# AnnaLew/pangenomix

Hardware: AMD Instinct MI355X
Metric: proteins/sec clustered at 0.8 identity + pan/core iters/sec, 400-genome set (higher is better)
Workload: dtype i32

## Files before the change

pangenomix_amd/csrc/cluster.hip:

```cpp
#include <algorithm>
#include <chrono>
#include <cstdlib>
#include <cmath>
#include <type_traits>
#include <functional>
#include <condition_variable>
#include <mutex>
#include <thread>
#include <vector>

#include "cluster_layout.h"
#include "cluster_resolve.h"
#include "cluster_tables.h"
#include "pgx_internal.h"

namespace {

using namespace pgxc;

constexpr uint32_t kWindowMax = 65536;
constexpr int kDiscoveryRounds = 2;
constexpr uint32_t kBlockCap = 4096;
constexpr uint32_t kBlockCapMin = 64;

// ... 39 lines not shown
    const uint8_t *res;
    const uint64_t *off;
    const uint32_t *len;
    const uint32_t *wcode;
    const uint16_t *wmult;
    const uint32_t *wcnt;
    const uint32_t *pk;
    const uint32_t *pk_off;
    uint32_t n_fwd;
    int32_t base;
    int32_t kd;
    int32_t nt;
    uint32_t mshift;
};
__device__ __forceinline__ uint32_t entry_rmask(const DevSeqs &S) { return (1u << S.mshift) - 1u; }
__device__ __forceinline__ uint32_t entry_fmax(const DevSeqs &S) { return 0xFFFFFFFFu >> S.mshift; }
__device__ __forceinline__ uint32_t real_of(const DevSeqs &S, uint32_t k) { return k >= S.n_fwd ? k - S.n_fwd : k; }

__constant__ int8_t kAa2Idx_dev[26] = {0, 2, 4, 3, 6, 13, 7, 8, 9, 20, 11, 10, 12,
                                       2, 20, 14, 5, 1, 15, 16, 20, 19, 17, 20, 18, 6};

__device__ __forceinline__ bool is_letter(uint8_t ch) {
    ch &= 0xDF;
    return ch >= 'A' && ch <= 'Z';
}

__global__ __launch_bounds__(256) void seq_len_kernel(const uint8_t *__restrict__ res,
                                                     const uint64_t *__restrict__ off, uint32_t n, uint64_t total,
                                                     uint32_t *__restrict__ len) {
    const uint32_t lane = threadIdx.x & 63u;
    const uint32_t i = blockIdx.x * 4u + (threadIdx.x >> 6);
    if (i >= n) return;
    const uint64_t b = off[i], e = off[i + 1];
    uint32_t c = 0;
    const uint64_t a0 = b & ~3ull;
    for (uint64_t a = a0 + 4ull * lane; a < e; a += 256) {
        uint32_t word = 0;
        if (a + 4 <= total) word = *reinterpret_cast<const uint32_t *>(res + a);
        else for (uint64_t p = a; p < total; ++p) word |= (uint32_t)res[p] << (8 * (p - a));
#pragma unroll
        for (int t = 0; t < 4; ++t) {
            const uint64_t p = a + t;
            c += (p >= b && p < e) && is_letter((uint8_t)(word >> (8 * t)));
        }
    }
    for (int d = 32; d > 0; d >>= 1) c += __shfl_xor(c, d);
    if (lane == 0) len[i] = c;
}

__global__ __launch_bounds__(256) void encode_gather_kernel(const uint8_t *__restrict__ in,
                                                           const uint64_t *__restrict__ in_off,
                                                           const uint32_t *__restrict__ order,
                                                           const uint64_t *__restrict__ out_off,
                                                           uint8_t *__restrict__ out, uint32_t n, int nt) {
    const uint32_t lane = threadIdx.x & 63u;
    const uint32_t k = blockIdx.x * 4u + (threadIdx.x >> 6);
    if (k >= n) return;
    const uint32_t src = order[k];
    const uint64_t b = in_off[src], e = in_off[src + 1];
    uint64_t w = out_off[k];
    for (uint64_t q0 = b; q0 < e; q0 += 256) {
        uint8_t chs[4];
#pragma unroll
        for (int j = 0; j < 4; ++j) { const uint64_t p = q0 + 64u * j + lane; chs[j] = p < e ? in[p] : (uint8_t)0; }
#pragma unroll
        for (int j = 0; j < 4; ++j) {
            const uint8_t ch = chs[j];
            const bool ok = is_letter(ch);
            const unsigned long long m = __ballot(ok);
            if (ok) {
                const uint8_t up = ch & 0xDF;
                const uint8_t idx = nt ? (uint8_t)(up == 'A' ? 0 : up == 'C' ? 1 : up == 'G' ? 2 : (up == 'T' || up == 'U') ? 3 : 4)
                                       : (uint8_t)kAa2Idx_dev[up - 'A'];
                out[w + __popcll(m & ((1ull << lane) - 1ull))] = idx;
            }
            w += __popcll(m);
        }
    }
}

__global__ __launch_bounds__(256) void revcomp_kernel(uint8_t *__restrict__ res, const uint64_t *__restrict__ off,
                                                     const uint32_t *__restrict__ len, uint32_t n) {
    const uint32_t lane = threadIdx.x & 63u;
    const uint32_t k = blockIdx.x * 4u + (threadIdx.x >> 6);
    if (k >= n) return;
    const uint64_t src = off[k], dst = off[n + k];
    const uint32_t L = len[k];
    for (uint32_t i = lane; i < L; i += 64) {
        const uint8_t b = res[src + L - 1 - i];
        res[dst + i] = b < 4 ? (uint8_t)(3 - b) : b;
    }
}

__global__ __launch_bounds__(256) void pack5_kernel(const uint8_t *__restrict__ res, const uint64_t *__restrict__ off,
                                                   const uint32_t *__restrict__ len,
                                                   const uint32_t *__restrict__ pk_off, uint32_t n,
                                                   uint32_t *__restrict__ pk) {
    const uint32_t lane = threadIdx.x & 63u;
    const uint32_t k = blockIdx.x * 4u + (threadIdx.x >> 6);
    if (k >= n) return;
    const uint8_t *s = res + off[k];
    const uint32_t L = len[k], nw = (L + 5u) / 6u;
    uint32_t *dst = pk + pk_off[k];
    for (uint32_t w = lane; w < nw; w += 64) {
        uint32_t x = 0;
        for (uint32_t t = 0; t < 6; ++t)
            if (6 * w + t < L) x |= (uint32_t)s[6 * w + t] << (5u * t);
        dst[w] = x;
    }
}

constexpr uint32_t kDevSortMaxLen = 65535;
constexpr uint32_t kHistLds = 4096;
constexpr uint32_t kSortShare = 1024;
constexpr uint32_t kSortCells = 4u << 20;
constexpr uint32_t kScanTile = 2048;
enum : uint32_t { H_OVER = 0, H_MAX = 1, H_BINS = 4 };

constexpr int kClearSegs = 6;
struct ClearArgs { uint32_t *p[kClearSegs]; uint32_t words[kClearSegs]; int n; uint32_t *one; };
__global__ __launch_bounds__(256) void clear_kernel(ClearArgs a) {
    const uint32_t t = blockIdx.x * 256u + threadIdx.x, step = gridDim.x * 256u;
    for (int s = 0; s < a.n; ++s)
        for (uint32_t i = t; i < a.words[s]; i += step) a.p[s][i] = 0u;
    if (a.one && t == 0) *a.one = 1u;
}

__global__ __launch_bounds__(1024) void len_hist_kernel(const uint32_t *__restrict__ len, uint32_t n, int32_t min_length,
                                                       uint32_t *__restrict__ hist) {
    __shared__ uint32_t h[kHistLds];
    for (uint32_t b = threadIdx.x; b < kHistLds; b += 1024u) h[b] = 0u;
    __syncthreads();
    uint32_t mx = 0, over = 0;
    for (uint32_t i = blockIdx.x * 1024u + threadIdx.x; i < n; i += gridDim.x * 1024u) {
        const uint32_t L = len[i];
        mx = max(mx, L);
        if (L > kDevSortMaxLen) { ++over; continue; }
        if ((int32_t)L <= min_length) continue;
        if (L < kHistLds) atomicAdd(&h[L], 1u);
        else atomicAdd(&hist[H_BINS + L], 1u);
    }
    for (int d = 32; d > 0; d >>= 1) { mx = max(mx, (uint32_t)__shfl_xor(mx, d)); over += __shfl_xor(over, d); }
    if ((threadIdx.x & 63u) == 0) {
        if (mx) atomicMax(&hist[H_MAX], mx);
        if (over) atomicAdd(&hist[H_OVER], over);
    }
    __syncthreads();
    for (uint32_t b = threadIdx.x; b < kHistLds; b += 1024u)
        if (h[b]) atomicAdd(&hist[H_BINS + b], h[b]);
}

__global__ __launch_bounds__(256) void sort_count_kernel(const uint32_t *__restrict__ len, uint32_t n, int32_t min_length,
                                                        uint32_t max_len, uint32_t per, uint32_t n_shares,
// ... 1888 lines not shown
    hipEvent_t strike = nullptr, post = nullptr;
    WindowSet(pgx_ctx *c, DevSlot counters, DevSlot best, DevSlot flags, DevSlot pairs, DevSlot gscratch, PinSlot w,
              PinSlot b, PinSlot cnt)
        : counters_buf(c, counters), best_buf(c, best), flags_buf(c, flags), pairs_buf(c, pairs), gscratch_buf(c, gscratch),
          hW(c, w), h_best(c, b), h_ccnt(c, cnt) {}
    WindowSet(const WindowSet &) = delete;
    WindowSet &operator=(const WindowSet &) = delete;
    ~WindowSet() {
        if (strike) (void)hipEventDestroy(strike);
        if (post) (void)hipEventDestroy(post);
    }
};

struct PendingWindow {
    bool pending = false;
    uint32_t b0 = 0, nb = 0, nW = 0;
    bool sweep = false;
    int set = 0;
    uint64_t window_words = 0;
    Pinned<Pair> *hW = nullptr;
    Pinned<unsigned long long> *h_best = nullptr;
    Pinned<uint32_t> *h_ccnt = nullptr;
};

struct ClusterCall {
    pgx_ctx *ctx;
    const pgx_cluster_params *P;
    hipStream_t st_main;
    const uint8_t *d_residues = nullptr;
    const uint64_t *d_offsets = nullptr;
    uint32_t n_in = 0;
    uint64_t total_in = 0;
    int32_t *out_cluster = nullptr, *out_member = nullptr;
    float *out_identity = nullptr;
    uint8_t *out_strand = nullptr;
    bool want_stats = false;
    bool nt, both, overlap, exchanging, native_exchange, count_replicated;
    uint32_t shard_index, shard_count;
    bool trace, trace2;
    unsigned nth = 1;
    Clock::time_point t_call0, t_loop0;
    double t_mark = 0.0, t_resolve = 0.0, t_close = 0.0;
    bool dev_sort = false, need_gscratch = false, chunking = false;
    uint32_t n = 0, nv = 0, max_len = 0, n_runs = 0, mshift = 8, n_codes = 1, bm_words = 0;
    uint32_t window_cap = 0, pair_cap_k = 0, packed_len = 0, diag_grid = 0, gs_stride = 0, gs_cells = 0, tag_stride = 1;
    uint64_t total = 0, total_pk = 0, max_window_words = 0;
    double thr_frac = 0.0;
    const uint32_t *len_hist = nullptr;
    std::vector<uint32_t> host_hist;
    uint64_t *run_off = nullptr;
    uint32_t *run_pos = nullptr, *run_pk = nullptr;
    std::vector<uint32_t> flush_at;
    DevSeqs DS{};
    uint32_t pair_cap = 4u << 20;
    uint32_t block_cap = 0;
    int pool_cur = 0;
    uint64_t pool_cap = 0;
    uint32_t epoch_idx = 0;
    uint32_t epoch_tag = 0;
    double cur_frac = 0.0;
    uint64_t chunk_words = 0;
    uint64_t pending_words = 0;
    PendingWindow pending;
    DevBuf d_res, d_off, d_len, d_wcode, d_wmult, d_wcnt, d_aa1, d_aas, d_aan, d_lines, d_pool[2], d_idx, d_newbits, d_touched,
        d_first, d_rcvis, d_visits, d_pairsK, d_blk_list, d_ulist, d_new_list, d_order, d_list, d_gather, d_pk, d_pkoff, d_thr,
        d_hugewords, d_xsend, d_xrecv,
        d_hist, d_sortcnt, d_tilesum, d_runs, d_in_len;
    WindowSet sets[2];
    unsigned long long *x_send = nullptr;
    const unsigned long long *x_recv = nullptr;
    HostVec<uint32_t> h_hist, order, h_len, h_wcnt;
    HostVec<uint64_t> h_off, h_runs;
    HostVec<int32_t> h_thr;
    HostVec<int32_t> cluster_of;
    HostVec<int32_t> iden_of;
    HostVec<uint8_t> strand_of;
    Pinned<Pair> hK, h_gather;
    Pinned<unsigned long long> h_rcvis;
    Pinned<uint32_t> h_cnt, h_blk, h_new, h_list, h_push;
    Pinned<uint8_t> h_taken;
    std::vector<uint32_t> rep_seq;
    std::vector<uint32_t> members;
    std::vector<uint8_t> status;
    std::vector<unsigned long long> winner_key;
    std::vector<uint32_t> order_k, rank_of, bucket_k, fill_k, flight;
    pgx_cluster_stats S{};
    uint64_t gpu_pairs = 0, gpu_aligned = 0, gpu_aligned_bytes = 0, filter_walk_words = 0;
    uint64_t visits_rc = 0, n_rounds = 0, n_blocks = 0;
    int inject_rank = -1;
    uint64_t inject_at = 0, n_exchanges = 0;

    ClusterCall(pgx_ctx *c, const pgx_cluster_params *p, hipStream_t stream)
        : ctx(c), P(p), st_main(stream),
          d_res(c, CL_SLOT_RES), d_off(c, CL_SLOT_OFF), d_len(c, CL_SLOT_LEN), d_wcode(c, CL_SLOT_WCODE), d_wmult(c, CL_SLOT_WMULT),
          d_wcnt(c, CL_SLOT_WCNT), d_aa1(c, CL_SLOT_AA1), d_aas(c, CL_SLOT_AAS), d_aan(c, CL_SLOT_AAN), d_lines(c, CL_SLOT_LINES),
          d_pool{{c, CL_SLOT_POOL0}, {c, CL_SLOT_POOL1}}, d_idx(c, CL_SLOT_IDX), d_newbits(c, CL_SLOT_NEWBITS),
          d_touched(c, CL_SLOT_TOUCHED), d_first(c, CL_SLOT_FIRST), d_rcvis(c, CL_SLOT_RCVIS), d_visits(c, CL_SLOT_VISITS),
          d_pairsK(c, CL_SLOT_PAIRS_K), d_blk_list(c, CL_SLOT_BLK_LIST), d_ulist(c, CL_SLOT_ULIST), d_new_list(c, CL_SLOT_NEW_LIST),
          d_order(c, CL_SLOT_ORDER), d_list(c, CL_SLOT_LIST), d_gather(c, CL_SLOT_GATHER), d_pk(c, CL_SLOT_PK),
          d_pkoff(c, CL_SLOT_PKOFF), d_thr(c, CL_SLOT_THR), d_hugewords(c, CL_SLOT_HUGEWORDS), d_xsend(c, CL_SLOT_XSEND),
          d_xrecv(c, CL_SLOT_XRECV), d_hist(c, CL_SLOT_HIST), d_sortcnt(c, CL_SLOT_SORTCNT), d_tilesum(c, CL_SLOT_TILESUM),
          d_runs(c, CL_SLOT_RUNS), d_in_len(c, CL_SLOT_IN_LEN),
          sets{{c, CL_SLOT_COUNTERS, CL_SLOT_BEST_OWN, CL_SLOT_FLAGS, CL_SLOT_PAIRS_W, CL_SLOT_GSCRATCH, CL_PIN_W, CL_PIN_BEST, CL_PIN_CCNT},
               {c, CL_SLOT_COUNTERS2, CL_SLOT_BEST2, CL_SLOT_FLAGS2, CL_SLOT_PAIRS_W2, CL_SLOT_GSCRATCH2, CL_PIN_W2, CL_PIN_BEST2, CL_PIN_CCNT2}},
          hK(c, CL_PIN_K), h_gather(c, CL_PIN_GATHER), h_rcvis(c, CL_PIN_RCVIS), h_cnt(c, CL_PIN_CNT), h_blk(c, CL_PIN_BLK),
          h_new(c, CL_PIN_NEW), h_list(c, CL_PIN_LIST), h_push(c, CL_PIN_PUSH), h_taken(c, CL_PIN_TAKEN) {
        nt = P->alphabet == 1;
        both = nt && P->both_strands != 0;
        native_exchange = !P->exchange && P->shard_count >= 1 && ctx->comm;
        exchanging = P->exchange || native_exchange;
        shard_count = P->shard_count > 0 ? (uint32_t)P->shard_count : 1u;
        shard_index = P->shard_count > 0 ? (uint32_t)P->shard_index : 0u;
        count_replicated = shard_index == 0;
        overlap = !nt && !std::getenv("PGX_NO_OVERLAP");
        const char *tr = std::getenv("PGX_TRACE");
        trace = tr != nullptr;
        trace2 = trace && tr[0] == '2';
        sets[0].st = st_main;
        sets[1].st = ctx->stream2;
        t_call0 = t_loop0 = Clock::now();
    }
    void phase(const char *what) {
        if (!trace) return;
        const double now = 1e3 * seconds_since(t_call0);
        fprintf(stderr, "[pgx] %-28s %8.2f ms\n", what, now - t_mark);
        t_mark = now;
    }
    void give_stats(pgx_cluster_stats *stats) const { if (stats) *stats = S; }
};

struct Window {
    uint32_t b0 = 0, nb = 0, ns = 0;
    bool sweep = false;
    bool mark_absent = false;
    int set = 0;
    uint32_t n_reps = 0;
    uint64_t window_words = 0, blocks_before = 0;
    int two_len = 0, a16_slot = 0;
    uint32_t *d_poolp = nullptr;
    Chunks chunks;
    FilterArgs FA{};
    Clock::time_point t_sweep0;
    bool older_reps = false;
    uint32_t n_listed = 0;
    uint32_t n_struck = 0;
    bool strike_recorded = false;
    uint32_t nW = 0;
};

double chunk_frac_default() {
    static const double chunk_frac = std::getenv("PGX_CHUNK_FRAC") ? std::atof(std::getenv("PGX_CHUNK_FRAC")) : 0.8;
    return chunk_frac;
}


int ensure_pool(ClusterCall &C, uint64_t entries, hipStream_t on) {
    const uint64_t need = 8 * entries + 4096;
    if (need <= C.pool_cap) return PGX_OK;
    if (need > 0xFFFFFFF0ull) { pgx_set_error("pgx_cluster_greedy: word index too large for 32-bit pool offsets"); return PGX_ERR_CAPACITY; }
    const uint64_t want = std::min<uint64_t>(0xFFFFFFF0ull, need + need / 2);
    DevBuf &nb_ = C.d_pool[C.pool_cur ^ 1];
    PGX_HIP(nb_.alloc(want * 4));
    if (C.pool_cap) PGX_HIP(hipMemcpyAsync(nb_.p, C.d_pool[C.pool_cur].p, C.pool_cap * 4, hipMemcpyDeviceToDevice, on));
    C.pool_cur ^= 1;
    C.pool_cap = want;
    return PGX_OK;
}

uint32_t form_window(const ClusterCall &C, uint32_t b0, Chunks &chunks, uint32_t limit) {
    return pgxc::form_window(C.h_len.data(), b0, limit, C.window_cap, C.chunking, C.chunk_words, chunks);
}

void account(ClusterCall &C, const Pair *pp, uint32_t cnt) {
    for (uint32_t i = 0; i < cnt; ++i) {
// ... 404 lines not shown
    PGX_HIP(C.d_aan.alloc((size_t)n * 4));
    PGX_HIP(C.d_lines.alloc((size_t)C.n_codes * sizeof(IndexLine)));
    PGX_HIP(hipMemsetAsync(C.d_lines.p, 0, (size_t)C.n_codes * sizeof(IndexLine), st_main));
    PGX_HIP(C.sets[0].best_buf.alloc((size_t)window_cap * 8));
    PGX_HIP(C.d_rcvis.alloc((size_t)window_cap * 8));
    PGX_HIP(C.d_blk_list.alloc((size_t)kBlockCap * 4));
    PGX_HIP(C.d_ulist.alloc((size_t)window_cap * 4));
    PGX_HIP(C.d_new_list.alloc((size_t)window_cap * 4));
    PGX_HIP(C.sets[0].flags_buf.alloc(4 * (size_t)window_cap));
    PGX_HIP(C.d_list.alloc((size_t)pair_cap_k * 4));
    PGX_HIP(C.d_gather.alloc((size_t)pair_cap_k * sizeof(Pair)));
    PGX_HIP(C.sets[0].pairs_buf.alloc((size_t)C.pair_cap * sizeof(Pair)));
    PGX_HIP(C.d_pairsK.alloc((size_t)pair_cap_k * sizeof(Pair)));
    if (C.need_gscratch) PGX_HIP(C.sets[0].gscratch_buf.alloc((size_t)C.diag_grid * C.gs_stride * 4));
    if (C.overlap) {
        if (!C.exchanging) PGX_HIP(C.sets[1].best_buf.alloc((size_t)window_cap * 8));
        PGX_HIP(C.sets[1].flags_buf.alloc(4 * (size_t)window_cap));
        PGX_HIP(C.sets[1].pairs_buf.alloc((size_t)C.pair_cap * sizeof(Pair)));
        if (C.need_gscratch) PGX_HIP(C.sets[1].gscratch_buf.alloc((size_t)C.diag_grid * C.gs_stride * 4));
    }
    PGX_HIP(C.d_order.alloc((size_t)n * 4));
    if (C.dev_sort) {
        uint32_t per = kSortShare;
        while ((uint64_t)((n_in + per - 1) / per) * n_runs > kSortCells) per *= 2;
        const uint32_t n_shares = (n_in + per - 1) / per, cells = n_shares * n_runs, tiles = (cells + kScanTile - 1) / kScanTile;
        PGX_HIP(C.d_sortcnt.alloc((size_t)cells * 4));
        PGX_HIP(C.d_tilesum.alloc((size_t)tiles * 4));
        uint32_t *const cnt = C.d_sortcnt.as<uint32_t>(), *const in_len = C.d_in_len.as<uint32_t>();
        ProfScope prof(ctx, "length_sort_kernels", st_main);
        ClearArgs ca{};
        ca.p[0] = cnt; ca.words[0] = cells; ca.n = 1;
        clear_kernel<<<std::min(2048u, (cells + 255u) / 256u), 256, 0, st_main>>>(ca);
        sort_count_kernel<<<(n_in + 255) / 256, 256, 0, st_main>>>(in_len, n_in, P->min_length, max_len, per, n_shares, cnt);
        tile_sum_kernel<<<tiles, 256, 0, st_main>>>(cnt, cells, C.d_tilesum.as<uint32_t>());
        tile_scan_kernel<<<tiles, 256, 0, st_main>>>(cnt, cells, C.d_tilesum.as<uint32_t>());
        sort_place_kernel<<<(n_shares + 3) / 4, 256, 0, st_main>>>(in_len, n_in, P->min_length, max_len, per, n_shares, cnt, n,
                                                                   C.d_order.as<uint32_t>());
        LAUNCH_CHECK();
        PGX_HIP(hipMemcpyAsync(C.order.data(), C.d_order.p, (size_t)n * 4, hipMemcpyDeviceToHost, st_main));
    } else {
        PGX_HIP(hipMemcpyAsync(C.d_order.p, C.order.data(), (size_t)n * 4, hipMemcpyHostToDevice, st_main));
    }
    {
        const size_t runs_bytes = 2 * ((size_t)n_runs + 1) * 8;
        PGX_HIP(C.d_runs.alloc(runs_bytes));
        PGX_HIP(hipMemcpyAsync(C.d_runs.p, C.h_runs.data(), runs_bytes, hipMemcpyHostToDevice, st_main));
        const uint64_t *const dr_off = C.d_runs.as<uint64_t>();
        const uint32_t *const dr_pos = reinterpret_cast<const uint32_t *>(dr_off + n_runs + 1), *const dr_pk = dr_pos + n_runs + 1;
        layout_kernel<<<nv / 256 + 1, 256, 0, st_main>>>(dr_off, dr_pos, dr_pk, n_runs, max_len, n, nv, C.d_len.as<uint32_t>(),
                                                         C.d_off.as<uint64_t>(), C.d_pkoff.as<uint32_t>());
        LAUNCH_CHECK();
    }
    {
        ProfScope prof(ctx, "encode_gather_kernel", st_main);
        encode_gather_kernel<<<(n + 3) / 4, 256, 0, st_main>>>(C.d_residues, C.d_offsets, C.d_order.as<uint32_t>(),
                                                               C.d_off.as<uint64_t>(), C.d_res.as<uint8_t>(), n, nt ? 1 : 0);
        if (both)
            revcomp_kernel<<<(n + 3) / 4, 256, 0, st_main>>>(C.d_res.as<uint8_t>(), C.d_off.as<uint64_t>(),
                                                             C.d_len.as<uint32_t>(), n);
        pack5_kernel<<<(nv + 3) / 4, 256, 0, st_main>>>(C.d_res.as<uint8_t>(), C.d_off.as<uint64_t>(), C.d_len.as<uint32_t>(),
                                                        C.d_pkoff.as<uint32_t>(), nv, C.d_pk.as<uint32_t>());
    }
    LAUNCH_CHECK();
    {
        PGX_HIP(C.d_thr.alloc(3 * ((size_t)max_len + 1) * 4));
        PGX_HIP(hipMemcpyAsync(C.d_thr.p, C.h_thr.data(), 3 * ((size_t)max_len + 1) * 4, hipMemcpyHostToDevice, st_main));
        thresholds_kernel<<<(n + 255) / 256, 256, 0, st_main>>>(C.d_len.as<uint32_t>(), n, C.d_thr.as<int32_t>(), max_len + 1,
                                                               C.d_aa1.as<int32_t>(), C.d_aas.as<int32_t>(), C.d_aan.as<int32_t>());
        LAUNCH_CHECK();
    }
    C.phase("alloc + sort + layout + encode (enq)");
    return PGX_OK;
}

int build_word_lists(ClusterCall &C) {
    pgx_ctx *ctx = C.ctx;
    const hipStream_t st_main = C.st_main;
    const bool nt = C.nt;
    const uint32_t n = C.n, max_len = C.max_len;
    const int wl = C.P->word_len;
    auto first_with_words_le = [&](uint32_t cap) { return pgxc::first_with_words_le(C.run_pos, max_len, cap, wl); };
    const uint32_t k32 = first_with_words_le(32768), k8 = first_with_words_le(8192),
                   k2 = first_with_words_le(2048), k1k = first_with_words_le(1023), k5 = first_with_words_le(512);
    int rc;
    uint8_t *r8 = C.d_res.as<uint8_t>(); uint64_t *o64 = C.d_off.as<uint64_t>(); uint32_t *l32 = C.d_len.as<uint32_t>();
    uint32_t *wc = C.d_wcode.as<uint32_t>(); uint16_t *wm = C.d_wmult.as<uint16_t>(); uint32_t *wn = C.d_wcnt.as<uint32_t>();
    const int base = nt ? 4 : kNAA1;
    for (uint32_t half = 0; half < (C.both ? 2u : 1u); ++half) {
        const uint32_t o = half * n;
        if (k32) {
            uint32_t slots = 65536;
            while (slots < 2u * max_len) slots *= 2;
            const uint32_t per_launch = std::min(k32, std::max(1u, (uint32_t)((256ull << 20) / ((uint64_t)slots * 8))));
            PGX_HIP(C.d_hugewords.alloc((size_t)per_launch * slots * 8));
            ProfScope prof(ctx, "words_kernel", st_main);
            for (uint32_t a = 0; a < k32; a += per_launch)
                words_huge_kernel<<<std::min(per_launch, k32 - a), 1024, 0, st_main>>>(r8, o64, l32, o + a, o + std::min(k32, a + per_launch), wl, base,
                                                                                        nt, C.d_hugewords.as<uint32_t>(), slots, wc, wm, wn,
                                                                                        C.sets[0].dc + C_ERR);
            LAUNCH_CHECK();
        }
        if ((rc = launch_words<32768, 1024>(ctx, st_main, r8, o64, l32, o + k32, o + k8, wl, base, nt, wc, wm, wn))) return rc;
        if ((rc = launch_words<8192, 1024>(ctx, st_main, r8, o64, l32, o + k8, o + k2, wl, base, nt, wc, wm, wn))) return rc;
        if ((rc = launch_words_hash<2048, 256>(ctx, st_main, r8, o64, l32, o + k2, o + k1k, wl, base, nt, wc, wm, wn))) return rc;
        if (k5 > k1k) {
            ProfScope prof(ctx, "words_kernel", st_main);
            words_wave_kernel<2048><<<(k5 - k1k + 3) / 4, 256, 0, st_main>>>(r8, o64, l32, o + k1k, o + k5, wl, base, nt, wc, wm, wn);
            LAUNCH_CHECK();
        }
        if (n > k5) {
            ProfScope prof(ctx, "words_kernel", st_main);
            words_wave_kernel<1024><<<(n - k5 + 3) / 4, 256, 0, st_main>>>(r8, o64, l32, o + k5, o + n, wl, base, nt, wc, wm, wn);
            LAUNCH_CHECK();
        }
    }
    C.DS = DevSeqs{C.d_res.as<uint8_t>(), C.d_off.as<uint64_t>(), C.d_len.as<uint32_t>(),
                   C.d_wcode.as<uint32_t>(), C.d_wmult.as<uint16_t>(), C.d_wcnt.as<uint32_t>(),
                   C.d_pk.as<uint32_t>(), C.d_pkoff.as<uint32_t>(), n, nt ? 4 : kNAA1, nt ? 4 : 2, nt ? 1 : 0, C.mshift};
    C.h_wcnt = HostVec<uint32_t>(ctx, CL_HOST_WCNT, n);
    CL_REQUIRE(C.h_wcnt.ok(), "out of host memory");
    PGX_HIP(hipMemcpyAsync(C.h_wcnt.data(), C.d_wcnt.p, (size_t)n * 4, hipMemcpyDeviceToHost, st_main));
    C.phase("word lists (enqueue)");
    return PGX_OK;
}

int plan_windows(ClusterCall &C) {
    pgx_ctx *ctx = C.ctx;
    const pgx_cluster_params *P = C.P;
    const uint32_t n = C.n, nv = C.nv, max_len = C.max_len, window_cap = C.window_cap;
    parallel_for(nv, C.nth, [&](unsigned, size_t b, size_t e) {
        expand_runs(C.run_off, C.run_pos, max_len, n, b, e, C.h_len.data(), C.h_off.data());
    });
    C.h_off[nv] = C.total;
    C.phase("host lengths + offsets");
    uint64_t max_window_words = 0;
    uint32_t max_chunks = 1;
    {
        Chunks chunks;
        size_t nf = 0;
        for (uint32_t b0 = 0, nbw; b0 < n; b0 += nbw) {
            while (nf < C.flush_at.size() && C.flush_at[nf] <= b0) ++nf;
            nbw = form_window(C, b0, chunks, nf < C.flush_at.size() ? C.flush_at[nf] : n);
            max_window_words = std::max<uint64_t>(max_window_words, C.h_off[b0 + nbw] - C.h_off[b0]);
            max_chunks = std::max(max_chunks, chunks.n);
        }
        if (!C.flush_at.empty())
            max_window_words = std::max<uint64_t>(max_window_words, C.h_off[std::min(n, window_cap)]);
    }
    if (C.chunking && C.flush_at.empty())
        max_window_words = std::max<uint64_t>(max_window_words,
            std::min<uint64_t>(C.h_off[std::min(n, window_cap)], (uint64_t)kMaxChunks * std::max<uint64_t>(C.chunk_words, max_len)));
    CL_REQUIRE(max_window_words < 0xFFFFFFF0ull, "window too large");
    C.max_window_words = max_window_words;
    PGX_HIP(C.d_touched.alloc((max_window_words + 16) * sizeof(Deferred)));
    if (C.chunking && n > window_cap / 2) max_chunks = kMaxChunks;
    while (C.tag_stride < max_chunks) C.tag_stride *= 2;
    PGX_HIP(C.d_first.alloc((size_t)C.tag_stride * C.n_codes * 4 + 16));
    C.cluster_of = HostVec<int32_t>(ctx, CL_HOST_CLUSTER_OF, n, -1);
    C.iden_of = HostVec<int32_t>(ctx, CL_HOST_IDEN_OF, n, -1);
    CL_REQUIRE(C.cluster_of.ok() && C.iden_of.ok(), "out of host memory");
    WindowSet &s0 = C.sets[0], &s1 = C.sets[1];
    PGX_HIP(s0.h_best.reserve(window_cap)); PGX_HIP(C.h_cnt.reserve(C_COUNT)); PGX_HIP(C.h_blk.reserve(kBlockCap));
    PGX_HIP(C.h_new.reserve(window_cap)); PGX_HIP(C.hK.reserve(C.pair_cap_k)); PGX_HIP(s0.hW.reserve(kPrefix));
    PGX_HIP(C.h_rcvis.reserve(window_cap)); PGX_HIP(C.h_push.reserve(2 * (size_t)window_cap + 4 * kBlockCap));
    PGX_HIP(C.h_list.reserve(C.pair_cap_k)); PGX_HIP(C.h_gather.reserve(C.pair_cap_k));
    PGX_HIP(s0.h_ccnt.reserve(C_COUNT));
    if (C.overlap) { PGX_HIP(s1.hW.reserve(kPrefix)); PGX_HIP(s1.h_best.reserve(window_cap)); PGX_HIP(s1.h_ccnt.reserve(C_COUNT)); }
    for (WindowSet &ws : C.sets) {
        PGX_HIP(hipEventCreateWithFlags(&ws.strike, hipEventDisableTiming));
        PGX_HIP(hipEventCreateWithFlags(&ws.post, hipEventDisableTiming));
    }
    if (C.native_exchange) {
        PGX_HIP(C.d_xsend.alloc((size_t)PGX_EXCHANGE_SLOTS * PGX_EXCHANGE_WORDS * 8));
        PGX_HIP(C.d_xrecv.alloc((size_t)PGX_EXCHANGE_SLOTS * C.shard_count * PGX_EXCHANGE_WORDS * 8));
    }
    C.x_send = C.native_exchange ? C.d_xsend.as<unsigned long long>() : static_cast<unsigned long long *>(P->exchange_send);
    C.x_recv = C.native_exchange ? C.d_xrecv.as<unsigned long long>() : static_cast<const unsigned long long *>(P->exchange_recv);
    for (int s = 0; s < (C.overlap ? 2 : 1); ++s) {
        WindowSet &ws = C.sets[s];
        ws.d_best = C.exchanging ? C.x_send + (size_t)s * PGX_EXCHANGE_WORDS : ws.best_buf.as<unsigned long long>();
        ws.d_done = ws.flags_buf.as<uint8_t>(); ws.d_inblk = ws.d_done + window_cap;
        ws.d_hascand = ws.d_done + 2 * (size_t)window_cap; ws.d_accepted = ws.d_done + 3 * (size_t)window_cap;
        ws.pairsW = ws.pairs_buf.as<Pair>();
        ws.d_gs = ws.gscratch_buf.as<uint32_t>();
    }
    if (const char *e = std::getenv("PGX_INJECT_ERROR")) { unsigned long long at = 0; if (sscanf(e, "%d:%llu", &C.inject_rank, &at) == 2) C.inject_at = at; else C.inject_rank = -1; }
    C.status.resize(window_cap);
    C.strand_of = HostVec<uint8_t>(ctx, CL_HOST_STRAND_OF, n, (uint8_t)0);
    CL_REQUIRE(C.strand_of.ok(), "out of host memory");
    C.winner_key.resize(window_cap);
    C.rank_of.resize(window_cap); C.bucket_k.resize(kBlockCap + 2); C.fill_k.resize(kBlockCap + 2);
    PGX_HIP(hipMemsetAsync(C.d_first.p, 0, (size_t)C.tag_stride * C.n_codes * 4, C.st_main));
    C.phase("window set-up");
    if (!C.flush_at.empty()) { PGX_HIP(C.h_taken.reserve(n)); std::fill(C.h_taken.p, C.h_taken.p + n, (uint8_t)0); }
    return PGX_OK;
}

int open_window(ClusterCall &C, WindowSet &ws, Window &W) {
    const uint32_t b0 = W.b0, nb = W.nb;
    if (C.overlap && C.S.sweeps > 0)
        PGX_HIP(hipStreamWaitEvent(ws.st, C.sets[W.set ^ 1].strike, 0));
    W.ns = C.both ? 2 * nb : nb;
    W.n_reps = (uint32_t)C.rep_seq.size();
    W.window_words = C.h_off[b0 + nb] - C.h_off[b0];
    { int rc = ensure_pool(C, C.S.rep_words + C.pending_words + W.window_words, ws.st); if (rc) return rc; }
    W.d_poolp = C.d_pool[C.pool_cur].as<uint32_t>();
    if (C.nt) {
        const uint64_t need = (uint64_t)W.ns * ((uint64_t)W.n_reps + nb) + 1024;
        if (need > (400ull << 20)) {
            pgx_set_error("pgx_cluster_greedy: %llu candidate pairs in one window exceed the supported maximum",
                          (unsigned long long)need);
            return PGX_ERR_CAPACITY;
        }
        if (need > C.pair_cap) {
            PGX_HIP(spin_sync(ws.st));
            { int rc = run_pending(C); if (rc) return rc; }
            C.pair_cap = (uint32_t)(need + need / 2);
            PGX_HIP(ws.pairs_buf.alloc((size_t)C.pair_cap * sizeof(Pair)));
            ws.pairsW = ws.pairs_buf.as<Pair>();
        }
    }
    C.S.sweeps++;
    W.t_sweep0 = Clock::now();
    W.blocks_before = C.n_blocks;
    W.two_len = 2 * (int)C.h_len[b0];
    const int two_len = W.two_len;
    W.a16_slot = two_len <= 1024 - 96 ? 1024 : (two_len <= 1536 - 96 ? 1536 : (two_len <= 2048 - 96 ? 2048 : (two_len <= 3072 - 96 ? 3072 : kA16MaxSlot)));
    unsigned long long *const d_rcvis = C.d_rcvis.as<unsigned long long>();
    FilterArgs &FA = W.FA;
    FA.lines = C.d_lines.as<IndexLine>(); FA.pool = W.d_poolp; FA.newbits = C.d_newbits.as<uint32_t>();
    FA.d_round_lo = ws.dc + C_SEG0; FA.d_round_hi = ws.dc + C_NEW; FA.epoch = 0;
    FA.b0 = b0; FA.nbq = nb; FA.ns = W.ns; FA.shard_index = C.shard_index; FA.shard_count = C.shard_count;
    FA.req_aan = C.d_aan.as<int32_t>(); FA.best = ws.d_best; FA.done = ws.d_done;
    FA.pairs = ws.pairsW; FA.n_pairs = ws.dc + C_NW; FA.pair_cap = C.pair_cap;
    FA.visits = C.d_visits.as<unsigned long long>(); FA.rc_visits = d_rcvis; FA.err = ws.dc + C_ERR;
    FA.qlist = nullptr; FA.d_nq = nullptr; FA.mark = nullptr; FA.count_visits = 1u;
    FA.lean = !C.want_stats && !std::getenv("PGX_NO_LEAN") ? 1u : 0u;

    window_init_kernel<<<(C.window_cap + 255) / 256, 256, 0, ws.st>>>(ws.dc, ws.d_best, C.both ? d_rcvis : nullptr, ws.d_done, C.window_cap);
    if (W.mark_absent)
        mark_absent_kernel<<<(nb + 255) / 256, 256, 0, ws.st>>>(C.h_taken.p + b0, nb, ws.d_done, ws.d_best);
    LAUNCH_CHECK();
    return PGX_OK;
}

int phase_a(ClusterCall &C, WindowSet &ws, Window &W) {
    {
        ProfScope prof(C.ctx, "filter_kernel<all>", ws.st);
        auto kern = C.nt ? filter_kernel<true, false> : filter_kernel<false, false>;
        kern<<<std::min(kFilterGrid, (W.ns + 3) / 4), 256, 0, ws.st>>>(C.DS, W.FA);
    }
    LAUNCH_CHECK();
    C.filter_walk_words += W.window_words * (C.both ? 2 : 1) / C.shard_count;
    W.older_reps = true;
// ... 184 lines not shown
}

int close_window(ClusterCall &C, WindowSet &ws, Window &W) {
    const hipStream_t st = ws.st;
    uint32_t *const dc = ws.dc;
    const uint32_t nb = W.nb;
    PubArgs pa{};
    pa.seg[0] = {dc, ws.h_ccnt.p, nullptr, C_COUNT, 1, C_COUNT};
    pa.seg[1] = {reinterpret_cast<const uint32_t *>(ws.d_best), reinterpret_cast<uint32_t *>(ws.h_best.p), nullptr, nb, 2, nb};
    pa.seg[2] = {reinterpret_cast<const uint32_t *>(ws.pairsW), reinterpret_cast<uint32_t *>(ws.hW.p), dc + C_NW, 0, kPairWords,
                 (uint32_t)std::min<size_t>(ws.hW.cap, C.pair_cap)};
    pa.n = 3;
    if (C.both) pa.seg[pa.n++] = {reinterpret_cast<const uint32_t *>(C.d_rcvis.as<unsigned long long>()), reinterpret_cast<uint32_t *>(C.h_rcvis.p), nullptr, nb, 2, nb};
    if (C.overlap && !W.strike_recorded) PGX_HIP(hipEventRecord(ws.strike, st));
    publish_kernel<<<64, 256, 0, st>>>(pa);
    LAUNCH_CHECK();
    if (C.overlap) PGX_HIP(hipEventRecord(ws.post, st));
    PendingWindow &pw = C.pending;
    pw.b0 = W.b0; pw.nb = nb; pw.nW = 0; pw.sweep = W.sweep; pw.set = W.set; pw.window_words = W.window_words;
    pw.hW = &ws.hW; pw.h_best = &ws.h_best; pw.h_ccnt = &ws.h_ccnt;
    if (!C.overlap) { int rc = wait_closed(C, pw); if (rc) return rc; W.nW = pw.nW; }
    const auto t_c0 = Clock::now();
    C.pending_words = W.window_words;
    pw.pending = true;
    if (C.nt || C.trace2) {
        int rc = run_pending(C); if (rc) return rc;
    }
    C.t_close += seconds_since(t_c0);
    return PGX_OK;
}

int finish_call(ClusterCall &C, uint32_t *out_n_clusters, pgx_cluster_stats *stats) {
    pgx_cluster_stats &S = C.S;
    if (C.trace) {
        const double loop_s = seconds_since(C.t_loop0);
        fprintf(stderr, "[pgx] windows %llu blocks %llu (+%llu follow-up rounds): loop %.1f ms = wait %.1f + block resolve %.1f + window close %.1f + "
                "enqueue/other %.1f\n", (unsigned long long)S.sweeps, (unsigned long long)C.n_blocks, (unsigned long long)C.n_rounds,
                1e3 * loop_s, 1e3 * g_wait_s, 1e3 * C.t_resolve, 1e3 * C.t_close,
                1e3 * (seconds_since(C.t_loop0) - g_wait_s - C.t_resolve - C.t_close));
    }
#ifdef PGX_FTIME
    {
        unsigned long long h[16], z[16] = {0};
        PGX_HIP(hipMemcpyFromSymbol(h, HIP_SYMBOL(g_ftime), sizeof h));
        PGX_HIP(hipMemcpyToSymbol(HIP_SYMBOL(g_ftime), z, sizeof z));
        static const char *nm[12] = {"prologue", "words+probes", "compaction", "last slab", "sync+reduce", "pass2 begin",
                                     "pass2 walk", "pass2 sync", "emit", "bucket clear", "kernel end", "-"};
        double tot = 0;
        for (int i = 0; i < 12; ++i) tot += (double)h[i];
        for (int i = 0; i < 11; ++i) fprintf(stderr, "[ftime] %-14s %6.2f %%\n", nm[i], 100.0 * (double)h[i] / tot);
        fprintf(stderr, "[ftime] %llu waves, %.0f clocks per wave; direct %llu, fallbacks %llu, classic %llu\n", h[12], tot / (double)h[12], h[13], h[14], h[15]);
    }
#endif
    if (C.overlap) PGX_HIP(hipStreamSynchronize(C.ctx->stream2));
    unsigned long long visits_table = 0;
    PGX_HIP(hipMemcpyAsync(&visits_table, C.d_visits.p, 8, hipMemcpyDeviceToHost, C.st_main));
    PGX_HIP(hipStreamSynchronize(C.st_main));
    S.posting_visits = visits_table + C.visits_rc;
    S.reserved[0] = C.gpu_pairs; S.reserved[1] = C.gpu_aligned; S.reserved[2] = C.gpu_aligned_bytes;
    S.reserved[3] = C.filter_walk_words;
    S.n_clusters = C.rep_seq.size();

    C.phase("window loop");
    if (out_n_clusters) *out_n_clusters = (uint32_t)C.rep_seq.size();
    C.give_stats(stats);
    return PGX_OK;
}

}

static int cluster_greedy_impl(pgx_ctx *ctx, const uint8_t *d_residues, const uint64_t *d_offsets,
                               uint32_t n_in, uint64_t total_in, const pgx_cluster_params *P,
                               int32_t *out_cluster, int32_t *out_member, float *out_identity,
                               uint8_t *out_strand, uint32_t *out_n_clusters,
                               pgx_cluster_stats *stats, void *stream_) {
    PGX_REQUIRE(ctx && P, "NULL argument");
    ClusterCall C(ctx, P, (hipStream_t)stream_);
    C.d_residues = d_residues; C.d_offsets = d_offsets; C.n_in = n_in; C.total_in = total_in;
    C.out_cluster = out_cluster; C.out_member = out_member; C.out_identity = out_identity; C.out_strand = out_strand;
    C.want_stats = stats != nullptr;
    int rc;
    if ((rc = check_params(C, out_cluster, out_member, out_identity))) return rc;
    C.t_call0 = Clock::now();
    C.S.n_input = n_in;
    if (out_n_clusters) *out_n_clusters = 0;
    C.nth = host_threads(n_in);
    parallel_for(n_in, C.nth, [&](unsigned, size_t b, size_t e) {
        for (size_t i = b; i < e; ++i) {
            out_cluster[i] = -1; out_member[i] = -1; out_identity[i] = 0.f;
            if (out_strand) out_strand[i] = 0;
        }
    });
    if (n_in == 0) { C.give_stats(stats); return PGX_OK; }
    if ((rc = order_by_length(C))) return rc;
    if (C.n == 0) { C.give_stats(stats); return PGX_OK; }
    if ((rc = prepare_input(C))) return rc;
    if ((rc = build_word_lists(C))) return rc;
    if ((rc = plan_windows(C))) return rc;

    C.t_loop0 = Clock::now();
    g_wait_s = 0.0;
    const std::vector<uint32_t> &flush_at = C.flush_at;
    const uint32_t n = C.n;
    size_t next_flush = 0;
    bool sweeping = false;
    uint32_t sweep_at = 0;
    for (uint32_t cursor = 0; cursor < n;) {
        if (!sweeping && next_flush < flush_at.size() && cursor == flush_at[next_flush]) {
            ++next_flush;
            sweeping = true; sweep_at = cursor;
            if ((rc = drain(C))) return rc;
        }
        Window W;
        W.sweep = sweeping;
        W.b0 = W.sweep ? sweep_at : cursor;
        W.nb = form_window(C, W.b0, W.chunks, W.sweep || next_flush >= flush_at.size() ? n : flush_at[next_flush]);
        W.mark_absent = !flush_at.empty() && next_flush > 0;
        W.set = C.overlap ? (int)(C.S.sweeps & 1u) : 0;
        WindowSet &ws = C.sets[W.set];
        if ((rc = open_window(C, ws, W))) return rc;
        if (W.b0 > 0 && (rc = phase_a(C, ws, W))) return rc;
        if (W.sweep) {
            if ((rc = begin_host_side(C, W))) return rc;
        } else {
            if ((rc = discovery_rounds(C, ws, W))) return rc;
            if ((rc = resolve_blocks(C, ws, W))) return rc;
        }
        adapt_chunks(C, W);
        if ((rc = close_window(C, ws, W))) return rc;
        if (C.trace2)
            fprintf(stderr, "[pgx] window %4llu b0 %8u nb %6u len %5u..%5u blocks %2llu reps +%5zu (discovery %5u) (total %7zu) pairs %7u  %.2f ms\n",
                    (unsigned long long)C.S.sweeps, W.b0, W.nb, C.h_len[W.b0], C.h_len[W.b0 + W.nb - 1],
                    (unsigned long long)(C.n_blocks - W.blocks_before), C.rep_seq.size() - W.n_reps, W.n_listed, C.rep_seq.size(), W.nW,
                    1e3 * seconds_since(W.t_sweep0));
        if (!W.sweep) { cursor += W.nb; continue; }
        sweep_at += W.nb;
        if (sweep_at >= n) {
            if ((rc = drain(C))) return rc;
            PGX_HIP(hipMemsetAsync(C.d_lines.p, 0, (size_t)C.n_codes * sizeof(IndexLine), C.st_main));
            const uint32_t one = 1u;
            PGX_HIP(hipMemcpyAsync(C.d_idx.p, &one, 4, hipMemcpyHostToDevice, C.st_main));
            PGX_HIP(hipStreamSynchronize(C.st_main));
            sweeping = false;
        }
    }
    if ((rc = run_pending(C))) return rc;
    return finish_call(C, out_n_clusters, stats);
}

extern "C" int pgx_cluster_greedy(pgx_ctx *ctx, const uint8_t *residues, const uint64_t *offsets,
// ... 22 lines not shown
```

pangenomix_amd/csrc/cluster_layout.h:

```cpp
#pragma once
#include <algorithm>
#include <cstddef>
#include <cstdint>

namespace pgxc {

inline uint64_t build_run_tables(const uint32_t *hist, uint32_t max_len, uint64_t *run_off, uint32_t *run_pos,
                                 uint32_t *run_pk) {
    const uint32_t n_runs = max_len + 1;
    uint64_t pos = 0, off = 0, pk = 0;
    for (uint32_t r = 0; r < n_runs; ++r) {
        run_pos[r] = (uint32_t)pos; run_off[r] = off; run_pk[r] = (uint32_t)pk;
        const uint64_t L = max_len - r, c = hist[L];
        pos += c; off += c * L; pk += c * ((L + 5) / 6);
    }
    run_pos[n_runs] = (uint32_t)pos; run_off[n_runs] = off; run_pk[n_runs] = (uint32_t)pk;
    return pk;
}

inline void expand_runs(const uint64_t *run_off, const uint32_t *run_pos, uint32_t max_len, uint32_t n, size_t b,
                        size_t e, uint32_t *len, uint64_t *off) {
    if (b >= e) return;
    const uint32_t n_runs = max_len + 1;
    size_t kk = b >= n ? b - n : b;
    uint32_t r = (uint32_t)(std::upper_bound(run_pos, run_pos + n_runs + 1, (uint32_t)kk) - run_pos) - 1;
    for (size_t k = b; k < e; ++k, ++kk) {
        if (kk == n) { kk = 0; r = 0; }
        while (run_pos[r + 1] <= kk) ++r;
        const uint32_t L = max_len - r;
        len[k] = L;
        off[k] = (k >= n ? run_off[n_runs] : 0) + run_off[r] + (uint64_t)(kk - run_pos[r]) * L;
    }
}

inline uint32_t first_with_words_le(const uint32_t *run_pos, uint32_t max_len, uint32_t cap, int word_len) {
    const uint64_t fits = (uint64_t)cap + (uint64_t)word_len - 1;
    return max_len > fits ? run_pos[max_len - (uint32_t)fits] : 0u;
}

}
```

Before: 16.64 million.

## Split sequence encoding and word-list build into head and overlapped tail slices

Encoding, reverse complement, 5-bit packing and word-list construction are no longer done for every sequence up front. Only the sequences needed by the first window are processed on the main stream. The remaining tail is enqueued on the second stream after a layout event, so the first clustering windows can run while the tail is still being prepared. Windows that reach past the head wait on a tail-ready event. The slice routine launches pack5 twice per slice, which is redundant work, and the extra events and stream dependencies add complexity.

```diff
diff --git a/pangenomix_amd/csrc/cluster.hip b/pangenomix_amd/csrc/cluster.hip
--- a/pangenomix_amd/csrc/cluster.hip
+++ b/pangenomix_amd/csrc/cluster.hip
@@ -115,10 +115,10 @@
                                                            const uint64_t *__restrict__ in_off,
                                                            const uint32_t *__restrict__ order,
                                                            const uint64_t *__restrict__ out_off,
-                                                           uint8_t *__restrict__ out, uint32_t n, int nt) {
+                                                           uint8_t *__restrict__ out, uint32_t k0, uint32_t k1, int nt) {
     const uint32_t lane = threadIdx.x & 63u;
-    const uint32_t k = blockIdx.x * 4u + (threadIdx.x >> 6);
-    if (k >= n) return;
+    const uint32_t k = k0 + blockIdx.x * 4u + (threadIdx.x >> 6);
+    if (k >= k1) return;
     const uint32_t src = order[k];
     const uint64_t b = in_off[src], e = in_off[src + 1];
     uint64_t w = out_off[k];
@@ -143,10 +143,10 @@
 }
 
 __global__ __launch_bounds__(256) void revcomp_kernel(uint8_t *__restrict__ res, const uint64_t *__restrict__ off,
-                                                     const uint32_t *__restrict__ len, uint32_t n) {
+                                                     const uint32_t *__restrict__ len, uint32_t n, uint32_t k0, uint32_t k1) {
     const uint32_t lane = threadIdx.x & 63u;
-    const uint32_t k = blockIdx.x * 4u + (threadIdx.x >> 6);
-    if (k >= n) return;
+    const uint32_t k = k0 + blockIdx.x * 4u + (threadIdx.x >> 6);
+    if (k >= k1) return;
     const uint64_t src = off[k], dst = off[n + k];
     const uint32_t L = len[k];
     for (uint32_t i = lane; i < L; i += 64) {
@@ -157,11 +157,11 @@
 
 __global__ __launch_bounds__(256) void pack5_kernel(const uint8_t *__restrict__ res, const uint64_t *__restrict__ off,
                                                    const uint32_t *__restrict__ len,
-                                                   const uint32_t *__restrict__ pk_off, uint32_t n,
+                                                   const uint32_t *__restrict__ pk_off, uint32_t k0, uint32_t k1,
                                                    uint32_t *__restrict__ pk) {
     const uint32_t lane = threadIdx.x & 63u;
-    const uint32_t k = blockIdx.x * 4u + (threadIdx.x >> 6);
-    if (k >= n) return;
+    const uint32_t k = k0 + blockIdx.x * 4u + (threadIdx.x >> 6);
+    if (k >= k1) return;
     const uint8_t *s = res + off[k];
     const uint32_t L = len[k], nw = (L + 5u) / 6u;
     uint32_t *dst = pk + pk_off[k];
@@ -2156,6 +2156,9 @@
     uint32_t *run_pos = nullptr, *run_pk = nullptr;
     std::vector<uint32_t> flush_at;
     DevSeqs DS{};
+    uint32_t head = 0;
+    bool tail_enqueued = false;
+    hipEvent_t laid_out = nullptr, tail_ready = nullptr;
     uint32_t pair_cap = 4u << 20;
     uint32_t block_cap = 0;
     int pool_cur = 0;
@@ -2224,6 +2227,12 @@
         sets[1].st = ctx->stream2;
         t_call0 = t_loop0 = Clock::now();
     }
+    ClusterCall(const ClusterCall &) = delete;
+    ClusterCall &operator=(const ClusterCall &) = delete;
+    ~ClusterCall() {
+        if (laid_out) (void)hipEventDestroy(laid_out);
+        if (tail_ready) (void)hipEventDestroy(tail_ready);
+    }
     void phase(const char *what) {
         if (!trace) return;
         const double now = 1e3 * seconds_since(t_call0);
@@ -2734,75 +2743,119 @@
         LAUNCH_CHECK();
     }
     {
-        ProfScope prof(ctx, "encode_gather_kernel", st_main);
-        encode_gather_kernel<<<(n + 3) / 4, 256, 0, st_main>>>(C.d_residues, C.d_offsets, C.d_order.as<uint32_t>(),
-                                                               C.d_off.as<uint64_t>(), C.d_res.as<uint8_t>(), n, nt ? 1 : 0);
-        if (both)
-            revcomp_kernel<<<(n + 3) / 4, 256, 0, st_main>>>(C.d_res.as<uint8_t>(), C.d_off.as<uint64_t>(),
-                                                             C.d_len.as<uint32_t>(), n);
-        pack5_kernel<<<(nv + 3) / 4, 256, 0, st_main>>>(C.d_res.as<uint8_t>(), C.d_off.as<uint64_t>(), C.d_len.as<uint32_t>(),
-                                                        C.d_pkoff.as<uint32_t>(), nv, C.d_pk.as<uint32_t>());
-    }
-    LAUNCH_CHECK();
-    {
         PGX_HIP(C.d_thr.alloc(3 * ((size_t)max_len + 1) * 4));
         PGX_HIP(hipMemcpyAsync(C.d_thr.p, C.h_thr.data(), 3 * ((size_t)max_len + 1) * 4, hipMemcpyHostToDevice, st_main));
         thresholds_kernel<<<(n + 255) / 256, 256, 0, st_main>>>(C.d_len.as<uint32_t>(), n, C.d_thr.as<int32_t>(), max_len + 1,
                                                                C.d_aa1.as<int32_t>(), C.d_aas.as<int32_t>(), C.d_aan.as<int32_t>());
         LAUNCH_CHECK();
     }
-    C.phase("alloc + sort + layout + encode (enq)");
+    PGX_HIP(hipEventCreateWithFlags(&C.laid_out, hipEventDisableTiming));
+    PGX_HIP(hipEventRecord(C.laid_out, st_main));
+    C.phase("alloc + sort + layout (enq)");
     return PGX_OK;
 }
 
-int build_word_lists(ClusterCall &C) {
+struct HugeWords { uint32_t slots = 0, per_launch = 0; };
+
+int enqueue_slice(ClusterCall &C, hipStream_t st, uint32_t lo, uint32_t hi, const uint32_t *bounds, const HugeWords &hw,
+                  uint32_t *err) {
+    if (hi <= lo) return PGX_OK;
     pgx_ctx *ctx = C.ctx;
-    const hipStream_t st_main = C.st_main;
     const bool nt = C.nt;
+    const uint32_t n = C.n, cnt = hi - lo;
+    const int wl = C.P->word_len, base = nt ? 4 : kNAA1;
+    uint8_t *r8 = C.d_res.as<uint8_t>(); uint64_t *o64 = C.d_off.as<uint64_t>(); uint32_t *l32 = C.d_len.as<uint32_t>();
+    uint32_t *wc = C.d_wcode.as<uint32_t>(); uint16_t *wm = C.d_wmult.as<uint16_t>(); uint32_t *wn = C.d_wcnt.as<uint32_t>();
+    const uint32_t halves = C.both ? 2u : 1u;
+    {
+        ProfScope prof(ctx, "encode_gather_kernel", st);
+        encode_gather_kernel<<<(cnt + 3) / 4, 256, 0, st>>>(C.d_residues, C.d_offsets, C.d_order.as<uint32_t>(), o64, r8, lo, hi,
+                                                            nt ? 1 : 0);
+        if (C.both) revcomp_kernel<<<(cnt + 3) / 4, 256, 0, st>>>(r8, o64, l32, n, lo, hi);
+        for (uint32_t half = 0; half < halves; ++half)
+            pack5_kernel<<<(cnt + 3) / 4, 256, 0, st>>>(r8, o64, l32, C.d_pkoff.as<uint32_t>(), half * n + lo, half * n + hi,
+                                                        C.d_pk.as<uint32_t>());
+    }
+    LAUNCH_CHECK();
+    pgxc::ClassLaunch launches[pgxc::WC_CLASSES];
+    const int n_launches = pgxc::class_launches(bounds, n, lo, hi, launches);
+    for (uint32_t half = 0; half < halves; ++half)
+        for (int i = 0; i < n_launches; ++i) {
+            const uint32_t a = half * n + launches[i].lo, b = half * n + launches[i].hi;
+            int rc = PGX_OK;
+            switch (launches[i].cls) {
+            case pgxc::WC_HUGE: {
+                ProfScope prof(ctx, "words_kernel", st);
+                for (uint32_t k = a; k < b; k += hw.per_launch)
+                    words_huge_kernel<<<std::min(hw.per_launch, b - k), 1024, 0, st>>>(r8, o64, l32, k, std::min(b, k + hw.per_launch), wl,
+                                                                                       base, nt, C.d_hugewords.as<uint32_t>(), hw.slots,
+                                                                                       wc, wm, wn, err);
+                break;
+            }
+            case pgxc::WC_LDS32K: rc = launch_words<32768, 1024>(ctx, st, r8, o64, l32, a, b, wl, base, nt, wc, wm, wn); break;
+            case pgxc::WC_LDS8K: rc = launch_words<8192, 1024>(ctx, st, r8, o64, l32, a, b, wl, base, nt, wc, wm, wn); break;
+            case pgxc::WC_HASH2K: rc = launch_words_hash<2048, 256>(ctx, st, r8, o64, l32, a, b, wl, base, nt, wc, wm, wn); break;
+            case pgxc::WC_WAVE2K: {
+                ProfScope prof(ctx, "words_kernel", st);
+                words_wave_kernel<2048><<<(b - a + 3) / 4, 256, 0, st>>>(r8, o64, l32, a, b, wl, base, nt, wc, wm, wn);
+                break;
+            }
+            default: {
+                ProfScope prof(ctx, "words_kernel", st);
+                words_wave_kernel<1024><<<(b - a + 3) / 4, 256, 0, st>>>(r8, o64, l32, a, b, wl, base, nt, wc, wm, wn);
+            }
+            }
+            if (rc) return rc;
+            LAUNCH_CHECK();
+        }
+    {
+        ProfScope prof(ctx, "encode_gather_kernel", st);
+        for (uint32_t half = 0; half < halves; ++half)
+            pack5_kernel<<<(cnt + 3) / 4, 256, 0, st>>>(r8, o64, l32, C.d_pkoff.as<uint32_t>(), half * n + lo, half * n + hi,
+                                                        C.d_pk.as<uint32_t>());
+    }
+    LAUNCH_CHECK();
+    PGX_HIP(hipMemcpyAsync(C.h_wcnt.data() + lo, wn + lo, (size_t)cnt * 4, hipMemcpyDeviceToHost, st));
+    return PGX_OK;
+}
+
+int build_sequences(ClusterCall &C) {
+    pgx_ctx *ctx = C.ctx;
     const uint32_t n = C.n, max_len = C.max_len;
     const int wl = C.P->word_len;
+    {
+        expand_runs(C.run_off, C.run_pos, max_len, n, 0, std::min(n, C.window_cap), C.h_len.data(), C.h_off.data());
+        Chunks chunks;
+        C.head = form_window(C, 0, chunks, C.flush_at.empty() ? n : C.flush_at[0]);
+        if (std::getenv("PGX_SERIAL_PROLOGUE")) C.head = n;
+    }
     auto first_with_words_le = [&](uint32_t cap) { return pgxc::first_with_words_le(C.run_pos, max_len, cap, wl); };
-    const uint32_t k32 = first_with_words_le(32768), k8 = first_with_words_le(8192),
-                   k2 = first_with_words_le(2048), k1k = first_with_words_le(1023), k5 = first_with_words_le(512);
-    int rc;
-    uint8_t *r8 = C.d_res.as<uint8_t>(); uint64_t *o64 = C.d_off.as<uint64_t>(); uint32_t *l32 = C.d_len.as<uint32_t>();
-    uint32_t *wc = C.d_wcode.as<uint32_t>(); uint16_t *wm = C.d_wmult.as<uint16_t>(); uint32_t *wn = C.d_wcnt.as<uint32_t>();
-    const int base = nt ? 4 : kNAA1;
-    for (uint32_t half = 0; half < (C.both ? 2u : 1u); ++half) {
-        const uint32_t o = half * n;
-        if (k32) {
-            uint32_t slots = 65536;
-            while (slots < 2u * max_len) slots *= 2;
-            const uint32_t per_launch = std::min(k32, std::max(1u, (uint32_t)((256ull << 20) / ((uint64_t)slots * 8))));
-            PGX_HIP(C.d_hugewords.alloc((size_t)per_launch * slots * 8));
-            ProfScope prof(ctx, "words_kernel", st_main);
-            for (uint32_t a = 0; a < k32; a += per_launch)
-                words_huge_kernel<<<std::min(per_launch, k32 - a), 1024, 0, st_main>>>(r8, o64, l32, o + a, o + std::min(k32, a + per_launch), wl, base,
-                                                                                        nt, C.d_hugewords.as<uint32_t>(), slots, wc, wm, wn,
-                                                                                        C.sets[0].dc + C_ERR);
-            LAUNCH_CHECK();
-        }
-        if ((rc = launch_words<32768, 1024>(ctx, st_main, r8, o64, l32, o + k32, o + k8, wl, base, nt, wc, wm, wn))) return rc;
-        if ((rc = launch_words<8192, 1024>(ctx, st_main, r8, o64, l32, o + k8, o + k2, wl, base, nt, wc, wm, wn))) return rc;
-        if ((rc = launch_words_hash<2048, 256>(ctx, st_main, r8, o64, l32, o + k2, o + k1k, wl, base, nt, wc, wm, wn))) return rc;
-        if (k5 > k1k) {
-            ProfScope prof(ctx, "words_kernel", st_main);
-            words_wave_kernel<2048><<<(k5 - k1k + 3) / 4, 256, 0, st_main>>>(r8, o64, l32, o + k1k, o + k5, wl, base, nt, wc, wm, wn);
-            LAUNCH_CHECK();
-        }
-        if (n > k5) {
-            ProfScope prof(ctx, "words_kernel", st_main);
-            words_wave_kernel<1024><<<(n - k5 + 3) / 4, 256, 0, st_main>>>(r8, o64, l32, o + k5, o + n, wl, base, nt, wc, wm, wn);
-            LAUNCH_CHECK();
-        }
+    const uint32_t bounds[pgxc::WC_CLASSES - 1] = {first_with_words_le(32768), first_with_words_le(8192), first_with_words_le(2048),
+                                                   first_with_words_le(1023), first_with_words_le(512)};
+    const uint32_t k32 = bounds[0], h = C.head;
+    HugeWords hw;
+    if (k32) {
+        hw.slots = 65536;
+        while (hw.slots < 2u * max_len) hw.slots *= 2;
+        hw.per_launch = std::min(k32, std::max(1u, (uint32_t)((256ull << 20) / ((uint64_t)hw.slots * 8))));
+        PGX_HIP(C.d_hugewords.alloc((size_t)hw.per_launch * hw.slots * 8));
     }
     C.DS = DevSeqs{C.d_res.as<uint8_t>(), C.d_off.as<uint64_t>(), C.d_len.as<uint32_t>(),
                    C.d_wcode.as<uint32_t>(), C.d_wmult.as<uint16_t>(), C.d_wcnt.as<uint32_t>(),
-                   C.d_pk.as<uint32_t>(), C.d_pkoff.as<uint32_t>(), n, nt ? 4 : kNAA1, nt ? 4 : 2, nt ? 1 : 0, C.mshift};
+                   C.d_pk.as<uint32_t>(), C.d_pkoff.as<uint32_t>(), n, C.nt ? 4 : kNAA1, C.nt ? 4 : 2, C.nt ? 1 : 0, C.mshift};
     C.h_wcnt = HostVec<uint32_t>(ctx, CL_HOST_WCNT, n);
     CL_REQUIRE(C.h_wcnt.ok(), "out of host memory");
-    PGX_HIP(hipMemcpyAsync(C.h_wcnt.data(), C.d_wcnt.p, (size_t)n * 4, hipMemcpyDeviceToHost, st_main));
-    C.phase("word lists (enqueue)");
+    { int rc = enqueue_slice(C, C.st_main, 0, h, bounds, hw, C.sets[0].dc + C_ERR); if (rc) return rc; }
+    if (h < n) {
+        const hipStream_t st2 = ctx->stream2;
+        PGX_HIP(hipEventCreateWithFlags(&C.tail_ready, hipEventDisableTiming));
+        PGX_HIP(hipEventRecord(C.laid_out, C.st_main));
+        PGX_HIP(hipStreamWaitEvent(st2, C.laid_out, 0));
+        C.tail_enqueued = true;
+        { int rc = enqueue_slice(C, st2, h, n, bounds, hw, C.sets[C.overlap ? 1 : 0].dc + C_ERR); if (rc) return rc; }
+        PGX_HIP(hipEventRecord(C.tail_ready, st2));
+    }
+    C.phase("encode + word lists (enqueue)");
     return PGX_OK;
 }
 
@@ -2882,6 +2935,8 @@
     const uint32_t b0 = W.b0, nb = W.nb;
     if (C.overlap && C.S.sweeps > 0)
         PGX_HIP(hipStreamWaitEvent(ws.st, C.sets[W.set ^ 1].strike, 0));
+    if (C.tail_enqueued && b0 + nb > C.head && ws.st != C.ctx->stream2)
+        PGX_HIP(hipStreamWaitEvent(ws.st, C.tail_ready, 0));
     W.ns = C.both ? 2 * nb : nb;
     W.n_reps = (uint32_t)C.rep_seq.size();
     W.window_words = C.h_off[b0 + nb] - C.h_off[b0];
@@ -3172,7 +3227,7 @@
         fprintf(stderr, "[ftime] %llu waves, %.0f clocks per wave; direct %llu, fallbacks %llu, classic %llu\n", h[12], tot / (double)h[12], h[13], h[14], h[15]);
     }
 #endif
-    if (C.overlap) PGX_HIP(hipStreamSynchronize(C.ctx->stream2));
+    if (C.overlap || C.tail_enqueued) PGX_HIP(hipStreamSynchronize(C.ctx->stream2));
     unsigned long long visits_table = 0;
     PGX_HIP(hipMemcpyAsync(&visits_table, C.d_visits.p, 8, hipMemcpyDeviceToHost, C.st_main));
     PGX_HIP(hipStreamSynchronize(C.st_main));
@@ -3215,7 +3270,7 @@
     if ((rc = order_by_length(C))) return rc;
     if (C.n == 0) { C.give_stats(stats); return PGX_OK; }
     if ((rc = prepare_input(C))) return rc;
-    if ((rc = build_word_lists(C))) return rc;
+    if ((rc = build_sequences(C))) return rc;
     if ((rc = plan_windows(C))) return rc;
 
     C.t_loop0 = Clock::now();
diff --git a/pangenomix_amd/csrc/cluster_layout.h b/pangenomix_amd/csrc/cluster_layout.h
--- a/pangenomix_amd/csrc/cluster_layout.h
+++ b/pangenomix_amd/csrc/cluster_layout.h
@@ -38,4 +38,19 @@
     return max_len > fits ? run_pos[max_len - (uint32_t)fits] : 0u;
 }
 
+enum WordClass : int { WC_HUGE = 0, WC_LDS32K, WC_LDS8K, WC_HASH2K, WC_WAVE2K, WC_WAVE1K, WC_CLASSES };
+struct ClassLaunch { int cls; uint32_t lo, hi; };
+
+inline int class_launches(const uint32_t bounds[WC_CLASSES - 1], uint32_t n, uint32_t lo, uint32_t hi,
+                          ClassLaunch out[WC_CLASSES]) {
+    int m = 0;
+    hi = std::min(hi, n);
+    for (int c = 0; c < WC_CLASSES; ++c) {
+        const uint32_t a = std::max(lo, c == 0 ? 0u : std::min(bounds[c - 1], n));
+        const uint32_t b = std::min(hi, c == WC_CLASSES - 1 ? n : std::min(bounds[c], n));
+        if (a < b) out[m++] = ClassLaunch{c, a, b};
+    }
+    return m;
 }
+
+}
```

New measurement: 16.75 million, median of 3. About the same (+0.7%).
